# MaverickPeter/MR_SLAM

Hardware: AMD Instinct MI355X
Metric: loop-candidate pairs/sec (BEV+Radon+corr), 120k-pt scans (higher is better)
Workload: dtype f32; 1 GPU; BASELINE configs[1] batched: 120k-pt synthetic lidar scans -> Cartesian BEV 120x120x1 -> Radon 120x120 -> normalise -> half spectrum -> FFT-domain rotation correlation vs 1 candidate of the database (+ 1 query per launch swept over the database)

## Files before the change

### mr_slam_amd/csrc/bev_cart.hpp

```cpp
#pragma once
#include "common.hpp"

namespace {

struct CartP {
    float gap_x, gap_y, gap_h;
    float inv_x, inv_y, inv_h;
    float eps_x, eps_y, eps_h;
    int NX, NY, H, F;
    float eps_fast;
};

__host__ __device__ inline float eps_for(int bins)
{
    float e = (float)(bins + 2) * 2e-6f;
    return e < 2e-4f ? 2e-4f : e;
}

__device__ __forceinline__ float cart_prep(float v)
{
    if (v == 0.0f) v = 0.0001f;
    if (v > 1.0f) v = 0.9999f;
    if (v < -1.0f) v = -0.9999f;
    return v;
}

__device__ __forceinline__ int cart_axis(float v, float gap, float inv, float eps)
{
    const float g = (v + 1.0f) * inv;
    const float f = floorf(g);
    const float fr = g - f;
    if (fr >= eps && fr <= 1.0f - eps) return (int)f;
    return (int)floor(((double)v + 1.0) / (double)gap);
}

__device__ __forceinline__ bool cart_cell(const CartP& p, float x, float y, float z, int& ix,
                                          int& iy, int& ih)
{
    x = cart_prep(x);
    y = cart_prep(y);
    z = cart_prep(z);
    if (!(x == x) || !(y == y) || !(z == z)) return false;
    ix = cart_axis(x, p.gap_x, p.inv_x, p.eps_x);
    iy = cart_axis(y, p.gap_y, p.inv_y, p.eps_y);
    ih = cart_axis(z, p.gap_h, p.inv_h, p.eps_h);
    return true;
}

__device__ __forceinline__ int cart_lin(const CartP& p, float x, float y, float z, int& col)
{
    int ix, iy, ih;
    if (!cart_cell(p, x, y, z, ix, iy, ih)) return -1;
    const long long cols = (long long)p.NX * p.NY;
    const long long c = (long long)iy + (long long)ix * p.NY;
    const long long lin = c + (long long)ih * cols;
    if (c < 0 || c >= cols || lin < 0 || lin >= cols * p.H) return -1;
    col = (int)c;
    return (int)lin;
}

__device__ __forceinline__ bool aligned16(const void* a) { return (((uintptr_t)a) & 15) == 0; }

typedef float f4v __attribute__((ext_vector_type(4)));
__device__ __forceinline__ float4 stream_load4(const float4* p)
{
    const f4v v = __builtin_nontemporal_load(reinterpret_cast<const f4v*>(p));
    return make_float4(v.x, v.y, v.z, v.w);
}
__device__ __forceinline__ void stream_store4(float4* p, float4 v)
{
    f4v w = {v.x, v.y, v.z, v.w};
    __builtin_nontemporal_store(w, reinterpret_cast<f4v*>(p));
}

inline int make_cart(const mrs_bev_cfg* c, bool feat, CartP& p)
{
    MRS_REQUIRE(c->n0 > 0 && c->n1 > 0 && c->num_height > 0, "grid sizes must be positive");
    MRS_REQUIRE(c->max_length > 0 && c->max_height > 0, "max_length / max_height must be positive");
    MRS_REQUIRE(!feat || c->enough_large >= 3, "featsize must be >= 3 (x,y,z planes)");
    MRS_REQUIRE((int64_t)c->n0 * c->n1 * c->num_height * (feat ? c->enough_large : 3) < (1ll << 28), "grid too large");
    MRS_REQUIRE(c->num_height <= 1024, "num_height > 1024 unsupported");
    p.NX = c->n0; p.NY = c->n1; p.H = c->num_height; p.F = feat ? c->enough_large : 3;
    p.gap_x = (float)(2.0 * (float)c->max_length / (float)c->n0);
    p.gap_y = (float)(2.0 * (float)c->max_length / (float)c->n1);
    p.gap_h = (float)(2.0 * (float)c->max_height / (float)c->num_height);
    p.inv_x = 1.0f / p.gap_x; p.inv_y = 1.0f / p.gap_y; p.inv_h = 1.0f / p.gap_h;
    p.eps_x = eps_for(p.NX); p.eps_y = eps_for(p.NY); p.eps_h = eps_for(p.H);
    p.eps_fast = (float)((p.NX > p.NY ? p.NX : p.NY) + 2) * 4e-7f;
    return MRS_OK;
}

}
```

### mr_slam_amd/csrc/fused.hip

```cpp
#include "common.hpp"
#include "bev_cart.hpp"
#include "radon_device.hpp"

#include <algorithm>
#include <cstdlib>

namespace {

template <int PF>
__device__ __forceinline__ void rasterise_scan(int* icells, int which, const float* __restrict__ px, const float* __restrict__ py,
                                               const float* __restrict__ pz, int n, const CartP& p, int stride)
{
    const float eps = p.eps_fast;
    const float inv_x = p.inv_x, inv_y = p.inv_y;
    const float fstride = (float)stride;
    const int NY = p.NY;
    int* const origin = icells + 2 * (kPad * stride + kPad) + which;
    auto prep = [&](float x, float y, float z, int& off, int& zi) {
        const float gx = __builtin_fmaf(x, inv_x, inv_x), gy = __builtin_fmaf(y, inv_y, inv_y);
        const float fx = floorf(gx), fy = floorf(gy);
        const float ex = 0.5f - fabsf((gx - fx) - 0.5f), ey = 0.5f - fabsf((gy - fy) - 0.5f);
        const bool fast = (bool)((int)(z > 0.0f) & (int)(z < 1.0f) & (int)(fabsf(x) <= 1.0f) & (int)(fabsf(y) <= 1.0f) & (int)(x * y != 0.0f) &
                                 (int)(ex >= eps) & (int)(ey >= eps));
        const int cell = (int)__builtin_fmaf(fx, fstride, fy);
        off = fast ? 2 * cell : 0;
        zi = fast ? __float_as_int(z) : 0;
        if (!fast && z > 0.0f) {
            int col;
            const int lin = cart_lin(p, x, y, z, col);
            if (lin >= 0) {
                const int ix = lin / NY, iy = lin - ix * NY;
                atomicMax(origin + 2 * (ix * stride + iy), __float_as_int(z));
            }
        }
    };
    auto put = [&](float x, float y, float z) {
        int off, zi;
        prep(x, y, z, off, zi);
        if (origin[off] < zi) atomicMax(origin + off, zi);
    };
    int done = 0;
    if (aligned16(px) && aligned16(py) && aligned16(pz)) {
        const int n4 = n >> 2;
        const float4* x4 = reinterpret_cast<const float4*>(px);
        const float4* y4 = reinterpret_cast<const float4*>(py);
        const float4* z4 = reinterpret_cast<const float4*>(pz);
        constexpr int kStage = PF * kRadonWG;
        const int stages = n4 / kStage;
        auto fetch = [&](int s, float4 (&A)[PF], float4 (&Bv)[PF], float4 (&Cv)[PF]) {
#pragma unroll
            for (int u = 0; u < PF; ++u) {
                const int k = s * kStage + u * kRadonWG + (int)threadIdx.x;
                A[u] = stream_load4(x4 + k); Bv[u] = stream_load4(y4 + k); Cv[u] = stream_load4(z4 + k);
            }
        };
        auto rasterise = [&](const float4 (&A)[PF], const float4 (&Bv)[PF], const float4 (&Cv)[PF]) {
            int off[4 * PF], zi[4 * PF], cur[4 * PF];
#pragma unroll
            for (int u = 0; u < PF; ++u) {
                prep(A[u].x, Bv[u].x, Cv[u].x, off[4 * u + 0], zi[4 * u + 0]);
                prep(A[u].y, Bv[u].y, Cv[u].y, off[4 * u + 1], zi[4 * u + 1]);
                prep(A[u].z, Bv[u].z, Cv[u].z, off[4 * u + 2], zi[4 * u + 2]);
                prep(A[u].w, Bv[u].w, Cv[u].w, off[4 * u + 3], zi[4 * u + 3]);
            }
#pragma unroll
            for (int k = 0; k < 4 * PF; ++k) cur[k] = origin[off[k]];
#pragma unroll
            for (int k = 0; k < 4 * PF; ++k)
                if (cur[k] < zi[k]) atomicMax(origin + off[k], zi[k]);
        };
        if (stages > 0) {
            float4 X[PF], Y[PF], Z[PF];
            fetch(0, X, Y, Z);
#pragma nounroll
            for (int s = 1; s < stages; ++s) {
                float4 Xn[PF], Yn[PF], Zn[PF];
                fetch(s, Xn, Yn, Zn);
                rasterise(X, Y, Z);
#pragma unroll
                for (int u = 0; u < PF; ++u) { X[u] = Xn[u]; Y[u] = Yn[u]; Z[u] = Zn[u]; }
            }
            rasterise(X, Y, Z);
        }
        for (int k = stages * kStage + (int)threadIdx.x; k < n4; k += kRadonWG) {
            const float4 A = stream_load4(x4 + k), Bv = stream_load4(y4 + k), Cv = stream_load4(z4 + k);
            put(A.x, Bv.x, Cv.x);
            put(A.y, Bv.y, Cv.y);
            put(A.z, Bv.z, Cv.z);
            put(A.w, Bv.w, Cv.w);
        }
        done = n4 << 2;
    }
    for (int i = done + threadIdx.x; i < n; i += kRadonWG) put(px[i], py[i], pz[i]);
}

template <int MAX_RAYS_PER_LANE, int STRIDE, int PF>
__global__ __launch_bounds__(kRadonWG) void k_bev_radon2(const float* __restrict__ xyz, const int64_t* __restrict__ offs, CartP cp, RadonP p,
                                                         int batch, float* __restrict__ bev_out, float* __restrict__ sino_raw,
                                                         float* __restrict__ sino_norm, int* __restrict__ degenerate,
                                                         unsigned* __restrict__ next_pair, unsigned stagger_ticks)
{
    extern __shared__ __attribute__((aligned(16))) int lds_i[];
    __shared__ double red[2][16];
    __shared__ unsigned s_next;
    const v2f* cells = reinterpret_cast<const v2f*>(lds_i);
    const int pairs = (batch + 1) >> 1;
    const int rows = p.H + 2 * kPad;
    const int rays = p.A * p.D;
    const int hw = p.H * p.W;
    if (stagger_ticks != 0u && (blockIdx.x & 1u)) {
        const unsigned long long t0 = wall_clock64();
        while (wall_clock64() - t0 < (unsigned long long)stagger_ticks) __builtin_amdgcn_s_sleep(64);
    }
    unsigned pair = blockIdx.x;
    while (pair < (unsigned)pairs) {
        int tid = (int)threadIdx.x;
        asm volatile("" : "+v"(tid));
        const int b0 = 2 * (int)pair, b1 = b0 + 1;
        const bool two = b1 < batch;
        int2* z2 = reinterpret_cast<int2*>(lds_i);
        for (int i = threadIdx.x; i < rows * p.stride; i += kRadonWG) z2[i] = make_int2(0, 0);
        __syncthreads();
        {
            const int64_t o = offs[b0];
            const int n = (int)(offs[b0 + 1] - o);
            const float* px = xyz + 3 * o;
            rasterise_scan<PF>(lds_i, 0, px, px + n, px + 2 * (size_t)n, n, cp, p.stride);
        }
        if (two) {
            const int64_t o = offs[b1];
            const int n = (int)(offs[b1 + 1] - o);
            const float* px = xyz + 3 * o;
            rasterise_scan<PF>(lds_i, 1, px, px + n, px + 2 * (size_t)n, n, cp, p.stride);
        }
        __syncthreads();
        if (bev_out) {
            for (int i = threadIdx.x; i < hw; i += kRadonWG) {
                const int y = i / p.W, x = i - y * p.W;
                const int2 c = z2[(y + kPad) * p.stride + x + kPad];
                bev_out[(size_t)b0 * hw + i] = __int_as_float(c.x);
                if (two) bev_out[(size_t)b1 * hw + i] = __int_as_float(c.y);
            }
        }
        float va[MAX_RAYS_PER_LANE], vb[MAX_RAYS_PER_LANE];
#pragma unroll
        for (int k = 0; k < MAX_RAYS_PER_LANE; ++k) {
            const int ray = tid + k * kRadonWG;
            float a = 0.0f, b = 0.0f;
            if (ray < rays) {
                trace_ray2<STRIDE>(cells, p, ray, a, b);
                if (sino_raw) {
                    sino_raw[(size_t)b0 * rays + ray] = a;
                    if (two) sino_raw[(size_t)b1 * rays + ray] = b;
                }
            }
            va[k] = a; vb[k] = b;
        }
        if (sino_norm) {
            normalize_store<MAX_RAYS_PER_LANE>(va, rays, red, sino_norm + (size_t)b0 * rays, degenerate);
            if (two) normalize_store<MAX_RAYS_PER_LANE>(vb, rays, red, sino_norm + (size_t)b1 * rays, degenerate);
        }
        __syncthreads();
        if (threadIdx.x == 0) s_next = gridDim.x + atomicAdd(next_pair, 1u);
        __syncthreads();
        pair = s_next;
    }
}


typedef float v16f __attribute__((ext_vector_type(16)));

template <int MAX_RAYS_PER_LANE, int STRIDE, int PF, bool ONCE = false>
__global__ __launch_bounds__(kRadonWG) void k_bev_radon3(const float* __restrict__ xyz, const int64_t* __restrict__ offs, CartP cp, RadonP p, SlotP sp,
                                                         int batch, float* __restrict__ bev_out, float* __restrict__ sino_raw,
                                                         float* __restrict__ sino_norm, float* __restrict__ park, int* __restrict__ degenerate,
                                                         unsigned* __restrict__ next_pair, unsigned stagger_ticks, int dev_skip)
{
    extern __shared__ __attribute__((aligned(16))) int lds_i[];
    __shared__ double red[2][16];
    __shared__ unsigned s_next;
    const v2f* cells = reinterpret_cast<const v2f*>(lds_i);
    const int pairs = (batch + 1) >> 1;
    const int rows = p.H + 2 * kPad;
    const int rays = p.A * p.D;
    const int hw = p.H * p.W;
    const unsigned tile0 = (unsigned)(uintptr_t)(lds_cptr)reinterpret_cast<const char*>(cells);
    if (stagger_ticks != 0u && (blockIdx.x & 1u)) {
        const unsigned long long t0 = wall_clock64();
        while (wall_clock64() - t0 < (unsigned long long)stagger_ticks) __builtin_amdgcn_s_sleep(64);
    }
    unsigned pair = blockIdx.x;
    while (pair < (unsigned)pairs) {
        int tid = (int)threadIdx.x;
        asm volatile("" : "+v"(tid));
        const int b0 = 2 * (int)pair, b1 = b0 + 1;
        const bool two = b1 < batch;
        int2* z2 = reinterpret_cast<int2*>(lds_i);
        for (int i = threadIdx.x; i < rows * p.stride; i += kRadonWG) z2[i] = make_int2(0, 0);
        __syncthreads();
        if (!(dev_skip & 1)) {
            const int64_t o = offs[b0];
            const int n = (int)(offs[b0 + 1] - o);
            const float* px = xyz + 3 * o;
            rasterise_scan<PF>(lds_i, 0, px, px + n, px + 2 * (size_t)n, n, cp, p.stride);
        }
        if (two && !(dev_skip & 1)) {
            const int64_t o = offs[b1];
            const int n = (int)(offs[b1 + 1] - o);
            const float* px = xyz + 3 * o;
            rasterise_scan<PF>(lds_i, 1, px, px + n, px + 2 * (size_t)n, n, cp, p.stride);
        }
        __syncthreads();
        if (bev_out) {
            for (int i = threadIdx.x; i < hw; i += kRadonWG) {
                const int y = i / p.W, x = i - y * p.W;
                const int2 c = z2[(y + kPad) * p.stride + x + kPad];
                bev_out[(size_t)b0 * hw + i] = __int_as_float(c.x);
                if (two) bev_out[(size_t)b1 * hw + i] = __int_as_float(c.y);
            }
        }
        float* const dA = sino_norm ? sino_norm + (size_t)b0 * rays : sino_raw ? sino_raw + (size_t)b0 * rays : park + (size_t)blockIdx.x * 2 * rays;
        float* const dB = sino_norm ? sino_norm + (size_t)b1 * rays : sino_raw ? sino_raw + (size_t)b1 * rays : dA + rays;
        float* const rA = sino_norm && sino_raw ? sino_raw + (size_t)b0 * rays : nullptr;
        int4 e = sp.slot[tid];
        float nrm = sp.nrm[tid];
        int ray = sp.ray[tid];
        const bool keep = ONCE && sino_norm != nullptr;
        v16f ka = 0.0f, kb = 0.0f;
#pragma nounroll
        for (int k = 0; k < MAX_RAYS_PER_LANE; ++k) {
            const int4 ce = e;
            const float cn = nrm;
            const int cr = ray;
            if (k + 1 < MAX_RAYS_PER_LANE) {
                const int s = tid + (k + 1) * kRadonWG;
                e = sp.slot[s]; nrm = sp.nrm[s]; ray = sp.ray[s];
            }
            const int n_steps = (dev_skip & 2) ? 0 : (ce.x & 0xffff);
            if (cr >= 0) {
                float a = 0.0f, b = 0.0f;
                if (n_steps > 0) {
                    const unsigned tile = tile0 + 2u * (unsigned)ce.y;
                    const float q = __int_as_float(ce.z), vm = __int_as_float(ce.w);
                    if (ce.x >> 16) march2<true, STRIDE>(tile, q, vm, n_steps, p.stride, a, b);
                    else march2<false, STRIDE>(tile, q, vm, n_steps, p.stride, a, b);
                    a *= cn; b *= cn;
                }
                if (keep) { ka[k] = a; kb[k] = b; }
                else {
                    dA[cr] = a;
                    if (two) dB[cr] = b;
                }
                if (rA) {
                    rA[cr] = a;
                    if (two) rA[rays + cr] = b;
                }
            }
        }
        __syncthreads();
        float* const tA = reinterpret_cast<float*>(lds_i);
        float* const tB = tA + rays;
        if (keep) {
#pragma unroll
            for (int k = 0; k < MAX_RAYS_PER_LANE; ++k) {
                const int cr = sp.ray[tid + k * kRadonWG];
                if (cr >= 0) { tA[cr] = ka[k]; tB[cr] = kb[k]; }
            }
            __syncthreads();
        }
        if (sino_norm) {
            float va[MAX_RAYS_PER_LANE], vb[MAX_RAYS_PER_LANE];
#pragma unroll
            for (int k = 0; k < MAX_RAYS_PER_LANE; ++k) {
                const int r = tid + k * kRadonWG;
                va[k] = r < rays ? (keep ? tA[r] : dA[r]) : 0.0f;
                vb[k] = (two && r < rays) ? (keep ? tB[r] : dB[r]) : 0.0f;
            }
            normalize_store<MAX_RAYS_PER_LANE>(va, rays, red, dA, degenerate, tid);
            if (two) normalize_store<MAX_RAYS_PER_LANE>(vb, rays, red, dB, degenerate, tid);
            __syncthreads();
        }
        if (threadIdx.x == 0) s_next = gridDim.x + atomicAdd(next_pair, 1u);
        __syncthreads();
        pair = s_next;
    }
}

template <int M, int S>
void* fused_kernel(int pf)
{
    return pf >= 4 ? reinterpret_cast<void*>(k_bev_radon2<M, S, 2>) : reinterpret_cast<void*>(k_bev_radon2<M, S, 1>);
}

template <int M, int S, bool ONCE = false>
void* fused_kernel_slots(int pf)
{
    return pf >= 6   ? reinterpret_cast<void*>(k_bev_radon3<M, S, 3, ONCE>)
           : pf >= 4 ? reinterpret_cast<void*>(k_bev_radon3<M, S, 2, ONCE>)
                     : reinterpret_cast<void*>(k_bev_radon3<M, S, 1, ONCE>);
}

}

extern "C" {

int mrs_radon_plan_set_option(mrs_radon_plan* plan, int32_t option, int32_t value)
{
    MRS_REQUIRE(plan, "null plan");
    switch (option) {
        case MRS_RADON_OPT_FUSED_STAGGER_US:
            MRS_REQUIRE(value >= 0 && value <= 100000, "stagger must be within [0, 100000] microseconds");
            plan->fused_stagger_us = value;
            return MRS_OK;
        case MRS_RADON_OPT_FUSED_PREFETCH:
            MRS_REQUIRE(value == 2 || value == 4 || value == 6, "prefetch depth must be 2, 4 or 6");
            plan->fused_prefetch = value;
            return MRS_OK;
        case MRS_RADON_OPT_FUSED_GRID:
            MRS_REQUIRE(value >= 0 && value <= 65535, "workgroup count must be within [0, 65535]");
            plan->fused_grid = value;
            return MRS_OK;
        case MRS_RADON_OPT_FUSED_VARIANT:
            MRS_REQUIRE(value >= 0 && value <= 2, "variant must be 0 (ray-order table, unrolled), 1 (slot tables) or 2 (slot tables, sinogram written once)");
            MRS_REQUIRE(value == 0 || plan->d_slot, "this plan has no slot tables");
            plan->fused_variant = value;
            return MRS_OK;
        case MRS_RADON_OPT_FUSED_SKIP:
            MRS_REQUIRE(value >= 0 && value <= 2, "skip must be 0 (run everything), 1 (no rasterising) or 2 (no ray march)");
            plan->fused_skip = value;
            return MRS_OK;
        default:
            mrs::set_error("unknown plan option %d", (int)option);
            return MRS_ERR_ARG;
    }
}

int mrs_ring_descriptors_batch(mrs_radon_plan* plan, const float* d_xyz, const int64_t* d_offsets, int32_t batch,
                               const mrs_bev_cfg* cfg, float* d_bev, float* d_sino, float* d_sino_norm, mrs_stream stream)
{
    MRS_REQUIRE(plan && d_xyz && d_offsets && cfg, "null pointer");
    MRS_REQUIRE(d_bev || d_sino || d_sino_norm, "at least one output required");
    MRS_REQUIRE(batch > 0, "batch must be positive");
    MRS_HIP_TRY(hipSetDevice(plan->ctx->device));
    CartP cp;
    int st = make_cart(cfg, false, cp);
    if (st != MRS_OK) return st;
    const int rays = plan->n_angles * plan->det;
    const int per_lane = (rays + kRadonWG - 1) / kRadonWG;
    if (cfg->num_height != 1 || cfg->n0 != plan->H || cfg->n1 != plan->W || !plan->two_in_lds || per_lane > 16) {
        mrs::set_error("fused descriptor kernel needs num_height == 1, a %d x %d grid (the plan's image), two images in the LDS and at most "
                       "16384 rays: run mrs_bev_cart_batch + mrs_radon_forward instead", plan->H, plan->W);
        return MRS_ERR_UNSUPPORTED;
    }
    RadonP p;
    p.A = plan->n_angles; p.D = plan->det; p.H = plan->H; p.W = plan->W;
    p.stride = (plan->W + 2 * kPad) | 1;
    const size_t nr = (size_t)p.A * p.D;
    p.meta = plan->d_meta;
    p.base = plan->d_meta + nr;
    p.q = reinterpret_cast<const float*>(plan->d_meta + 2 * nr);
    p.vm = p.q + nr;
    p.nrm = p.vm + nr;
    const size_t lds = 2 * (size_t)(p.H + 2 * kPad) * p.stride * sizeof(float);
    hipStream_t s = (hipStream_t)stream;
    mrs::Scratch ctr;
    if ((st = ctr.alloc(256, s)) != MRS_OK) return st;
    MRS_HIP_TRY(hipMemsetAsync(ctr.p, 0, sizeof(unsigned), s));
    const int pf = plan->fused_prefetch;
    const int pairs = (batch + 1) / 2;
    const int grid = std::min(pairs, plan->fused_grid > 0 ? plan->fused_grid : std::max(plan->ctx->num_cu, 1));
    unsigned stagger_ticks = (unsigned)plan->fused_stagger_us * 100u;
    if (pairs <= grid) stagger_ticks = 0;
    unsigned* d_ctr = ctr.as<unsigned>();
    int* d_deg = plan->d_degenerate;
    if (plan->fused_variant >= 1 && plan->d_slot && plan->slot_per_lane == per_lane) {
        const bool once = plan->fused_variant == 2 && 2 * (size_t)rays * sizeof(float) <= lds;
        void* kern = once ? (per_lane <= 15 ? (p.stride == 125 ? fused_kernel_slots<15, 125, true>(pf) : fused_kernel_slots<15, 0, true>(pf))
                                            : fused_kernel_slots<16, 0, true>(pf))
                          : (per_lane <= 15 ? (p.stride == 125 ? fused_kernel_slots<15, 125>(pf) : fused_kernel_slots<15, 0>(pf))
                                            : fused_kernel_slots<16, 0>(pf));
        if (lds > 48 * 1024) MRS_HIP_TRY(hipFuncSetAttribute(kern, hipFuncAttributeMaxDynamicSharedMemorySize, (int)lds));
        SlotP sp;
        sp.slot = plan->d_slot; sp.nrm = plan->d_slot_nrm; sp.ray = plan->d_slot_ray;
        mrs::Scratch parkbuf;
        float* d_park = nullptr;
        if (!d_sino && !d_sino_norm) {
            if ((st = parkbuf.alloc((size_t)grid * 2 * rays * sizeof(float), s)) != MRS_OK) return st;
            d_park = parkbuf.as<float>();
        }
        int dev_skip = plan->fused_skip;
        void* args[] = {(void*)&d_xyz, (void*)&d_offsets, (void*)&cp, (void*)&p, (void*)&sp, (void*)&batch, (void*)&d_bev, (void*)&d_sino,
                        (void*)&d_sino_norm, (void*)&d_park, (void*)&d_deg, (void*)&d_ctr, (void*)&stagger_ticks, (void*)&dev_skip};
        MRS_HIP_TRY(hipLaunchKernel(kern, dim3(grid), dim3(kRadonWG), args, lds, s));
        return MRS_OK;
    }
    void* kern = per_lane <= 15 ? (p.stride == 125 ? fused_kernel<15, 125>(pf) : fused_kernel<15, 0>(pf)) : fused_kernel<16, 0>(pf);
    if (lds > 48 * 1024) MRS_HIP_TRY(hipFuncSetAttribute(kern, hipFuncAttributeMaxDynamicSharedMemorySize, (int)lds));
    void* args[] = {(void*)&d_xyz, (void*)&d_offsets, (void*)&cp, (void*)&p, (void*)&batch, (void*)&d_bev, (void*)&d_sino,
                    (void*)&d_sino_norm, (void*)&d_deg, (void*)&d_ctr, (void*)&stagger_ticks};
    MRS_HIP_TRY(hipLaunchKernel(kern, dim3(grid), dim3(kRadonWG), args, lds, s));
    return MRS_OK;
}

}
```

Measured before the change: 2.342 million pairs/s.

## Bin BEV points with fixed-point float-bit arithmetic in slot kernel rasteriser

Adds a fixed-point binning path for Cartesian BEV rasterisation. An FMA with a power-of-two offset places the cell index and fractional guard bits directly in the float mantissa, so cell index, bounds check and edge-epsilon test become integer bit operations, and LDS addresses are computed directly with umul24. The slots kernel also gets a double-buffered prefetch loop and a compile-time stride of 125. The slots path is now used only when the host-side validity check for this trick passes, otherwise the code falls back, which risks a different kernel being selected for other configurations.

```diff
diff --git a/mr_slam_amd/csrc/bev_cart.hpp b/mr_slam_amd/csrc/bev_cart.hpp
--- a/mr_slam_amd/csrc/bev_cart.hpp
+++ b/mr_slam_amd/csrc/bev_cart.hpp
@@ -1,5 +1,6 @@
 #pragma once
 #include "common.hpp"
+#include "cart_fixed.hpp"
 
 namespace {
 
@@ -9,6 +10,11 @@
     float eps_x, eps_y, eps_h;
     int NX, NY, H, F;
     float eps_fast;
+    float fx_cx, fx_cy;
+    uint32_t fx_basex, fx_basey, fx_limx, fx_limy, fx_maskx, fx_masky, fx_g2;
+    int fx_Fx, fx_Fy;
+    int fx_zero;
+    int fx_mode;
 };
 
 __host__ __device__ inline float eps_for(int bins)
@@ -87,6 +93,15 @@
     p.inv_x = 1.0f / p.gap_x; p.inv_y = 1.0f / p.gap_y; p.inv_h = 1.0f / p.gap_h;
     p.eps_x = eps_for(p.NX); p.eps_y = eps_for(p.NY); p.eps_h = eps_for(p.H);
     p.eps_fast = (float)((p.NX > p.NY ? p.NX : p.NY) + 2) * 4e-7f;
+    const mrs::CartFixAxis ax = mrs::make_cart_fix(p.NX, p.inv_x), ay = mrs::make_cart_fix(p.NY, p.inv_y);
+    p.fx_cx = ax.c; p.fx_cy = ay.c;
+    p.fx_basex = ax.base; p.fx_basey = ay.base;
+    p.fx_limx = ax.lim; p.fx_limy = ay.lim;
+    p.fx_maskx = ax.mask; p.fx_masky = ay.mask;
+    p.fx_g2 = ax.g2;
+    p.fx_Fx = ax.F; p.fx_Fy = ay.F;
+    p.fx_zero = ax.zero_ok | ay.zero_ok;
+    p.fx_mode = !(ax.valid && ay.valid && ax.g2 == ay.g2) ? 0 : (ax.F == 16 && ay.F == 16 && !p.fx_zero) ? 2 : 1;
     return MRS_OK;
 }
 
diff --git a/mr_slam_amd/csrc/cart_fixed.hpp b/mr_slam_amd/csrc/cart_fixed.hpp
--- /dev/null
+++ b/mr_slam_amd/csrc/cart_fixed.hpp
@@ -0,0 +1,81 @@
+#pragma once
+#include <cmath>
+#include <cstdint>
+#include <cstring>
+
+#ifndef MRS_HD
+#if defined(__HIPCC__)
+#define MRS_HD __host__ __device__ __forceinline__
+#else
+#define MRS_HD inline
+#endif
+#endif
+
+namespace mrs {
+
+struct CartFixAxis {
+    float inv, c;
+    uint32_t base;
+    uint32_t lim;
+    uint32_t mask;
+    uint32_t g2;
+    int32_t F, G;
+    int32_t zero_ok;
+    int32_t valid;
+    float bound;
+};
+
+MRS_HD uint32_t fix_bits(float f)
+{
+#if defined(__HIP_DEVICE_COMPILE__)
+    return __float_as_uint(f);
+#else
+    uint32_t u;
+    memcpy(&u, &f, 4);
+    return u;
+#endif
+}
+
+MRS_HD uint32_t fix_w(float v, float inv, float c, uint32_t base) { return fix_bits(fmaf(v, inv, c)) - base; }
+
+template <bool F16>
+MRS_HD bool fix_ok(uint32_t w, uint32_t lim, uint32_t mask, uint32_t g2)
+{
+    if (F16) return (w < lim) & ((uint16_t)w >= (uint16_t)g2);
+    return (w < lim) & ((w & mask) >= g2);
+}
+
+MRS_HD bool fix_z01(uint32_t zbits) { return zbits - 1u < 0x3F7FFFFFu; }
+MRS_HD bool fix_zpos(uint32_t zbits) { return zbits - 1u < 0x7F800000u; }
+
+inline CartFixAxis make_cart_fix(int bins, float inv, int G = -1)
+{
+    CartFixAxis a;
+    memset(&a, 0, sizeof a);
+    int lg = 0;
+    while ((1 << lg) <= bins) ++lg;
+    const int M = 1 << lg;
+    a.F = 23 - lg;
+    a.G = G >= 0 ? G : 4;
+    a.inv = inv;
+    const double cd = (double)inv + (double)M;
+    a.c = (float)cd;
+    const float fM = (float)M;
+    uint32_t bM, bi;
+    memcpy(&bM, &fM, 4);
+    memcpy(&bi, &inv, 4);
+    a.base = bM - (uint32_t)a.G;
+    if (a.F < 1) return a;
+    a.lim = (uint32_t)bins << a.F;
+    a.mask = (1u << a.F) - 1u;
+    a.g2 = 2u * (uint32_t)a.G;
+    const double unit = ldexp(1.0, -a.F);
+    const double half_ulp_inv = ldexp(1.0, (int)((bi >> 23) & 0xff) - 127 - 24);
+    a.bound = (float)(2.0 * half_ulp_inv / unit + ((double)a.c == cd ? 0.0 : 0.5) + 0.5);
+    const uint32_t w0 = fix_bits(a.c) - a.base;
+    a.zero_ok = (w0 < a.lim) && ((w0 & a.mask) >= a.g2);
+    a.valid = a.F >= 14 && inv > 0.0f && inv < fM && (double)a.G >= 3.0 * (double)a.bound;
+    return a;
+}
+
+}
diff --git a/mr_slam_amd/csrc/fused.hip b/mr_slam_amd/csrc/fused.hip
--- a/mr_slam_amd/csrc/fused.hip
+++ b/mr_slam_amd/csrc/fused.hip
@@ -7,16 +7,27 @@
 
 namespace {
 
-template <int PF>
+typedef __attribute__((address_space(3))) int* lds_iptr;
+
+template <int PF, int FX, int STRIDE>
 __device__ __forceinline__ void rasterise_scan(int* icells, int which, const float* __restrict__ px, const float* __restrict__ py,
-                                               const float* __restrict__ pz, int n, const CartP& p, int stride)
-{
+                                               const float* __restrict__ pz, int n, const CartP& p, int rt_stride)
+{
+    const int stride = STRIDE > 0 ? STRIDE : rt_stride;
+    const int NY = p.NY;
+    int* const origin = icells + 2 * (kPad * stride + kPad) + which;
+    auto exact = [&](float x, float y, float z) {
+        int col;
+        const int lin = cart_lin(p, x, y, z, col);
+        if (lin >= 0) {
+            const int ix = lin / NY, iy = lin - ix * NY;
+            atomicMax(origin + 2 * (ix * stride + iy), __float_as_int(z));
+        }
+    };
     const float eps = p.eps_fast;
     const float inv_x = p.inv_x, inv_y = p.inv_y;
     const float fstride = (float)stride;
-    const int NY = p.NY;
-    int* const origin = icells + 2 * (kPad * stride + kPad) + which;
-    auto prep = [&](float x, float y, float z, int& off, int& zi) {
+    auto prep_float = [&](float x, float y, float z, int& off, int& zi) {
         const float gx = __builtin_fmaf(x, inv_x, inv_x), gy = __builtin_fmaf(y, inv_y, inv_y);
         const float fx = floorf(gx), fy = floorf(gy);
         const float ex = 0.5f - fabsf((gx - fx) - 0.5f), ey = 0.5f - fabsf((gy - fy) - 0.5f);
@@ -25,62 +36,108 @@
         const int cell = (int)__builtin_fmaf(fx, fstride, fy);
         off = fast ? 2 * cell : 0;
         zi = fast ? __float_as_int(z) : 0;
-        if (!fast && z > 0.0f) {
-            int col;
-            const int lin = cart_lin(p, x, y, z, col);
-            if (lin >= 0) {
-                const int ix = lin / NY, iy = lin - ix * NY;
-                atomicMax(origin + 2 * (ix * stride + iy), __float_as_int(z));
-            }
-        }
+        if (!fast && z > 0.0f) exact(x, y, z);
+    };
+    float cx = p.fx_cx, cy = p.fx_cy;
+    asm volatile("" : "+v"(cx), "+v"(cy));
+    const uint32_t bx = p.fx_basex, by = p.fx_basey, limx = p.fx_limx, limy = p.fx_limy, mx = p.fx_maskx, my = p.fx_masky, g2 = p.fx_g2;
+    const int Fx = FX == 2 ? 16 : p.fx_Fx, Fy = FX == 2 ? 16 : p.fx_Fy;
+    const bool zero_free = FX == 2 || p.fx_zero == 0;
+    const unsigned stride8 = 8u * (unsigned)stride;
+    const unsigned obase = (unsigned)(uintptr_t)(lds_cptr)reinterpret_cast<const char*>(origin);
+    auto cell_ptr = [](unsigned addr) { return (int*)(lds_iptr)(uintptr_t)addr; };
+    auto prep_fixed = [&](float x, float y, float z, unsigned& addr, int& zi) -> bool {
+        const uint32_t wx = mrs::fix_w(x, inv_x, cx, bx), wy = mrs::fix_w(y, inv_y, cy, by);
+        const uint32_t zb = __float_as_uint(z);
+        bool fast = (int)mrs::fix_ok<FX == 2>(wx, limx, mx, g2) & (int)mrs::fix_ok<FX == 2>(wy, limy, my, g2) & (int)mrs::fix_z01(zb);
+        if (FX != 2) fast = (int)fast & ((int)zero_free | (int)(x * y != 0.0f));
+        unsigned iy8 = (wy >> (Fy - 3)) & ~7u;
+        asm("" : "+v"(iy8));
+        const unsigned a = __umul24(wx >> Fx, stride8) + obase + iy8;
+        addr = fast ? a : obase;
+        zi = (int)zb;
+        if (!fast && mrs::fix_zpos(zb)) exact(x, y, z);
+        return fast;
+    };
+    auto prep = [&](float x, float y, float z, unsigned& addr, int& zi) -> bool {
+        if (FX == 0) {
+            int off;
+            prep_float(x, y, z, off, zi);
+            addr = obase + 4u * (unsigned)off;
+            return true;
+        }
+        return prep_fixed(x, y, z, addr, zi);
     };
     auto put = [&](float x, float y, float z) {
-        int off, zi;
-        prep(x, y, z, off, zi);
-        if (origin[off] < zi) atomicMax(origin + off, zi);
+        unsigned addr;
+        int zi;
+        const bool fast = prep(x, y, z, addr, zi);
+        if ((int)fast & (int)(*cell_ptr(addr) < zi)) atomicMax(cell_ptr(addr), zi);
     };
     int done = 0;
-    if (aligned16(px) && aligned16(py) && aligned16(pz)) {
+    if (aligned16(px) && aligned16(py) && aligned16(pz) && n < (1 << 28)) {
         const int n4 = n >> 2;
         const float4* x4 = reinterpret_cast<const float4*>(px);
         const float4* y4 = reinterpret_cast<const float4*>(py);
         const float4* z4 = reinterpret_cast<const float4*>(pz);
         constexpr int kStage = PF * kRadonWG;
         const int stages = n4 / kStage;
-        auto fetch = [&](int s, float4 (&A)[PF], float4 (&Bv)[PF], float4 (&Cv)[PF]) {
+        unsigned voff = (unsigned)threadIdx.x * 16u;
+        auto fetch = [&](float4 (&A)[PF], float4 (&Bv)[PF], float4 (&Cv)[PF]) {
 #pragma unroll
             for (int u = 0; u < PF; ++u) {
-                const int k = s * kStage + u * kRadonWG + (int)threadIdx.x;
-                A[u] = stream_load4(x4 + k); Bv[u] = stream_load4(y4 + k); Cv[u] = stream_load4(z4 + k);
-            }
+                const size_t o = (size_t)(voff + (unsigned)(u * kRadonWG * 16));
+                A[u] = stream_load4(reinterpret_cast<const float4*>(reinterpret_cast<const char*>(x4) + o));
+                Bv[u] = stream_load4(reinterpret_cast<const float4*>(reinterpret_cast<const char*>(y4) + o));
+                Cv[u] = stream_load4(reinterpret_cast<const float4*>(reinterpret_cast<const char*>(z4) + o));
+            }
+            voff += (unsigned)(kStage * 16);
         };
         auto rasterise = [&](const float4 (&A)[PF], const float4 (&Bv)[PF], const float4 (&Cv)[PF]) {
-            int off[4 * PF], zi[4 * PF], cur[4 * PF];
+            unsigned addr[4 * PF];
+            int zi[4 * PF], cur[4 * PF];
+            bool fast[4 * PF];
 #pragma unroll
             for (int u = 0; u < PF; ++u) {
-                prep(A[u].x, Bv[u].x, Cv[u].x, off[4 * u + 0], zi[4 * u + 0]);
-                prep(A[u].y, Bv[u].y, Cv[u].y, off[4 * u + 1], zi[4 * u + 1]);
-                prep(A[u].z, Bv[u].z, Cv[u].z, off[4 * u + 2], zi[4 * u + 2]);
-                prep(A[u].w, Bv[u].w, Cv[u].w, off[4 * u + 3], zi[4 * u + 3]);
-            }
-#pragma unroll
-            for (int k = 0; k < 4 * PF; ++k) cur[k] = origin[off[k]];
+                fast[4 * u + 0] = prep(A[u].x, Bv[u].x, Cv[u].x, addr[4 * u + 0], zi[4 * u + 0]);
+                fast[4 * u + 1] = prep(A[u].y, Bv[u].y, Cv[u].y, addr[4 * u + 1], zi[4 * u + 1]);
+                fast[4 * u + 2] = prep(A[u].z, Bv[u].z, Cv[u].z, addr[4 * u + 2], zi[4 * u + 2]);
+                fast[4 * u + 3] = prep(A[u].w, Bv[u].w, Cv[u].w, addr[4 * u + 3], zi[4 * u + 3]);
+            }
+#pragma unroll
+            for (int k = 0; k < 4 * PF; ++k) cur[k] = *cell_ptr(addr[k]);
 #pragma unroll
             for (int k = 0; k < 4 * PF; ++k)
-                if (cur[k] < zi[k]) atomicMax(origin + off[k], zi[k]);
+                if ((int)fast[k] & (int)(cur[k] < zi[k])) atomicMax(cell_ptr(addr[k]), zi[k]);
         };
-        if (stages > 0) {
+        if (FX == 0 && stages > 0) {
             float4 X[PF], Y[PF], Z[PF];
-            fetch(0, X, Y, Z);
+            fetch(X, Y, Z);
 #pragma nounroll
             for (int s = 1; s < stages; ++s) {
                 float4 Xn[PF], Yn[PF], Zn[PF];
-                fetch(s, Xn, Yn, Zn);
+                fetch(Xn, Yn, Zn);
                 rasterise(X, Y, Z);
 #pragma unroll
                 for (int u = 0; u < PF; ++u) { X[u] = Xn[u]; Y[u] = Yn[u]; Z[u] = Zn[u]; }
             }
             rasterise(X, Y, Z);
+        }
+        if (FX != 0 && stages > 0) {
+            float4 X0[PF], Y0[PF], Z0[PF], X1[PF], Y1[PF], Z1[PF];
+            fetch(X0, Y0, Z0);
+            int s = 0;
+#pragma nounroll
+            for (; s + 2 < stages; s += 2) {
+                fetch(X1, Y1, Z1);
+                rasterise(X0, Y0, Z0);
+                fetch(X0, Y0, Z0);
+                rasterise(X1, Y1, Z1);
+            }
+            const bool two_left = s + 2 == stages;
+            if (two_left) fetch(X1, Y1, Z1);
+            rasterise(X0, Y0, Z0);
+            if (two_left) rasterise(X1, Y1, Z1);
         }
         for (int k = stages * kStage + (int)threadIdx.x; k < n4; k += kRadonWG) {
             const float4 A = stream_load4(x4 + k), Bv = stream_load4(y4 + k), Cv = stream_load4(z4 + k);
@@ -125,13 +182,13 @@
             const int64_t o = offs[b0];
             const int n = (int)(offs[b0 + 1] - o);
             const float* px = xyz + 3 * o;
-            rasterise_scan<PF>(lds_i, 0, px, px + n, px + 2 * (size_t)n, n, cp, p.stride);
+            rasterise_scan<PF, 0, 0>(lds_i, 0, px, px + n, px + 2 * (size_t)n, n, cp, p.stride);
         }
         if (two) {
             const int64_t o = offs[b1];
             const int n = (int)(offs[b1 + 1] - o);
             const float* px = xyz + 3 * o;
-            rasterise_scan<PF>(lds_i, 1, px, px + n, px + 2 * (size_t)n, n, cp, p.stride);
+            rasterise_scan<PF, 0, 0>(lds_i, 1, px, px + n, px + 2 * (size_t)n, n, cp, p.stride);
         }
         __syncthreads();
         if (bev_out) {
@@ -202,13 +259,13 @@
             const int64_t o = offs[b0];
             const int n = (int)(offs[b0 + 1] - o);
             const float* px = xyz + 3 * o;
-            rasterise_scan<PF>(lds_i, 0, px, px + n, px + 2 * (size_t)n, n, cp, p.stride);
+            rasterise_scan<PF, STRIDE == 125 ? 2 : 1, STRIDE == 125 ? 125 : 0>(lds_i, 0, px, px + n, px + 2 * (size_t)n, n, cp, p.stride);
         }
         if (two && !(dev_skip & 1)) {
             const int64_t o = offs[b1];
             const int n = (int)(offs[b1 + 1] - o);
             const float* px = xyz + 3 * o;
-            rasterise_scan<PF>(lds_i, 1, px, px + n, px + 2 * (size_t)n, n, cp, p.stride);
+            rasterise_scan<PF, STRIDE == 125 ? 2 : 1, STRIDE == 125 ? 125 : 0>(lds_i, 1, px, px + n, px + 2 * (size_t)n, n, cp, p.stride);
         }
         __syncthreads();
         if (bev_out) {
@@ -373,11 +430,12 @@
     if (pairs <= grid) stagger_ticks = 0;
     unsigned* d_ctr = ctr.as<unsigned>();
     int* d_deg = plan->d_degenerate;
-    if (plan->fused_variant >= 1 && plan->d_slot && plan->slot_per_lane == per_lane) {
+    if (plan->fused_variant >= 1 && plan->d_slot && plan->slot_per_lane == per_lane && cp.fx_mode != 0) {
+        const bool s125 = p.stride == 125 && cp.fx_mode == 2;
         const bool once = plan->fused_variant == 2 && 2 * (size_t)rays * sizeof(float) <= lds;
-        void* kern = once ? (per_lane <= 15 ? (p.stride == 125 ? fused_kernel_slots<15, 125, true>(pf) : fused_kernel_slots<15, 0, true>(pf))
+        void* kern = once ? (per_lane <= 15 ? (s125 ? fused_kernel_slots<15, 125, true>(pf) : fused_kernel_slots<15, 0, true>(pf))
                                             : fused_kernel_slots<16, 0, true>(pf))
-                          : (per_lane <= 15 ? (p.stride == 125 ? fused_kernel_slots<15, 125>(pf) : fused_kernel_slots<15, 0>(pf))
+                          : (per_lane <= 15 ? (s125 ? fused_kernel_slots<15, 125>(pf) : fused_kernel_slots<15, 0>(pf))
                                             : fused_kernel_slots<16, 0>(pf));
         if (lds > 48 * 1024) MRS_HIP_TRY(hipFuncSetAttribute(kern, hipFuncAttributeMaxDynamicSharedMemorySize, (int)lds));
         SlotP sp;
```

After: 2.341 million pairs/s. Within noise of the previous version (-0.0%).
